# facebookresearch/vggsfm

Hardware: AMD Instinct MI355X
Metric: BA LM-iterations/sec (higher is better)
Workload: dtype f64

## Files before the change

vggsfm_amd/csrc/ba.hip:

```cpp
#include <type_traits>

#include "camera_model.hpp"
#include "../../include/vggsfm_amd.h"

namespace vgg {

int cholesky_solve_enqueue(double* A, double* b, int n, double* inv_blocks, int32_t* device_fail, const int32_t* skip_flag,
                           hipStream_t st, const CholOverlap* overlap, int split_a, int split_b, const int32_t* first_blk,
                           bool flags_cleared);
int32_t* cholesky_dataflow_flags(double* ws, int n, size_t* count);
size_t cholesky_workspace_bytes(int n);
void dataflow_signal(int32_t* flag, hipStream_t st);

constexpr int kGroup = 16;
#ifndef VGG_OFFDIAG_OCC
#define VGG_OFFDIAG_OCC 3
#endif
#ifndef VGG_DIAG_OCC
#define VGG_DIAG_OCC 4
#endif
#ifndef VGG_TILE_INTERLEAVE
#define VGG_TILE_INTERLEAVE 1
#endif
#ifndef VGG_DIAG_FULL_DEPTH
// ... 59 lines not shown
  double *scale_c, *scale_p, *colsq_c, *dsq_c, *dy;
  uint8_t* active;
  double* lin;
  double *U, *g, *costc;
  double* sys;
  double *S, *rhs;
  double* S2;
  double* gmax_pts;
  double* stepsum;
  double *G, *hs, *Ms;
  double *pdamp;
  double* T;
  double* part_B;
  double* part_F;
  double* packed;
  size_t packed_count;
  double* pk_mine;
  double* pk_gathered;
  double* cam_part;
  double* cam_split;
  double* Y;
  size_t y_bytes;
  double* chol_inv;
  double* tile_part;
  int32_t* batch_flags;
  double *Zp, *rz_part, *part_Q;
  unsigned long long* split_off;
  double* rz;
  int tile_rhs;
  int step_from_factors;
  double* Yx;
  size_t yx_bytes;
  int tile_dma;
  size_t lin_count, sys_count, total_bytes;
};

static inline size_t align_up(size_t x, size_t a) { return (x + a - 1) / a * a; }


static Dims make_dims(const vgg_ba_problem* pb) {
  Dims d;
  d.C = pb->num_cams; d.P = pb->num_pts; d.O = pb->num_obs; d.NI = pb->num_intr; d.model = pb->camera_model;
  const int rf = pb->refine_focal ? 1 : 0, rk = (pb->refine_extra && pb->camera_model == kSimpleRadial) ? 1 : 0;
  d.kd = rf + rk;
  d.only_k = (!rf && rk) ? 1 : 0;
  d.shared = (pb->num_intr == 1) ? 1 : 0;
  d.BDp = 6 + d.kd;
  d.n_red = 6 * d.C + d.kd * d.NI;
  d.kdsh = d.shared ? d.kd : 0;
  d.loss = pb->loss; d.loss_scale = pb->loss_scale;
  return d;
}

struct Tuning { int lpp, longt, cam_wgs, point_wgs, tile_rhs, step_factors, tile_dma; };
static Tuning g_tuning = [] {
  auto env = [](const char* name, int dflt) { const char* e = getenv(name); return e ? atoi(e) : dflt; };
  return Tuning{env("VGG_LPP", 0), env("VGG_PP_LONGT", -1), env("VGG_CAM_WGS", 0), env("VGG_POINT_WGS", 0), env("VGG_TILE_RHS", 2), env("VGG_STEP_FACTORS", 0), env("VGG_TILE_DMA", 0)};
}();

static Ws carve(const Dims& d, int max_iters, int num_chunks, int num_segments, void* base) {
  Ws w;
  size_t off = 0;
  auto take = [&](size_t bytes) { size_t o = off; off = align_up(off + bytes, 256); return (char*)base + o; };
  w.ctl = (Ctl*)take(sizeof(Ctl));
  w.log = (vgg_ba_iteration*)take(sizeof(vgg_ba_iteration) * (size_t)(max_iters + 2));
  w.cand_q = (double*)take(8ull * 4 * d.C); w.cand_t = (double*)take(8ull * 3 * d.C);
// ... 9 lines not shown
  w.sys = (double*)take(8ull * w.sys_count);
  w.S = w.sys; w.rhs = w.S + (size_t)d.n_red * d.n_red;
  w.S2 = (double*)take(8ull * (size_t)d.n_red * d.n_red);
  w.packed_count = (size_t)d.n_red * (d.n_red + 1) / 2 + d.n_red;
  w.packed = (double*)take(8ull * (w.packed_count + 2 * kPackPad));
  w.pk_mine = (double*)take(8ull * (w.packed_count + 2));
  w.pk_gathered = (double*)take(8ull * (w.packed_count + 3 * kPackPad));
  w.gmax_pts = (double*)take(64);
  w.stepsum = (double*)take(64);
  w.G = (double*)take(8ull * 6 * d.P); w.hs = (double*)take(8ull * 3 * d.P);
  w.pdamp = (double*)take(8ull * 3 * d.P);
  w.Ms = (double*)take(8ull * 3 * (d.kdsh ? d.kdsh : 1) * d.P);
  w.T = (double*)take(8ull * d.C * d.BDp * (1 + d.kdsh));
  w.part_B = (double*)take(8ull * kMaxWG);
  w.part_F = (double*)take(8ull * kMaxWG * 4);
  w.cam_part = (double*)take(8ull * (d.C + 1) * 3);
  w.cam_split = (double*)take(8ull * (size_t)d.C * kCamSplitMax * kCamNV);
  w.y_bytes = 8ull * ((size_t)(num_segments > 0 ? num_segments : 0) + 1) * kGroup * y_slot_doubles(d);
  w.Y = (double*)take(w.y_bytes);
  w.yx_bytes = (g_tuning.tile_dma && (d.shared || d.kd == 0)) ? 8ull * ((size_t)(num_segments > 0 ? num_segments : 0) + 1) * kGroup * 18 : 0;
  w.Yx = w.yx_bytes ? (double*)take(w.yx_bytes) : nullptr;
  w.tile_dma = 0;
  w.chol_inv = (double*)take(cholesky_workspace_bytes(d.n_red));
  {
    const size_t bdt = d.shared ? 6 : d.BDp;
    w.tile_part = (double*)take(8ull * (size_t)(num_chunks > 0 ? num_chunks : 1) * bdt * bdt * 256);
  }
  w.batch_flags = (int32_t*)take(64);
  w.Zp = (double*)take(8ull * 9 * (d.P > 0 ? d.P : 1));
  w.rz_part = (double*)take(8ull * (size_t)(num_chunks > 0 ? num_chunks : 1) * kGroup * 6 * 3);
  w.part_Q = (double*)take(8ull * kMaxWG * 8);
  w.rz = (double*)take(8ull * (size_t)((d.C + kGroup - 1) / kGroup) * kGroup * 6 * 3);
  w.split_off = (unsigned long long*)take(8ull * 2 * ((size_t)d.n_red + 2));
  w.tile_rhs = 0;
  w.total_bytes = off;
  return w;
}

struct DevProblem {
  Dims d;
  const double *cam_q, *cam_t, *intr, *pts;
  const int32_t *row_ptr, *obs_cam, *col_ptr, *cobs_pt, *obs_slot;
  const float2 *obs_uv, *cobs_uv;
  const uint8_t *cam_const, *intr_const, *pt_const;
};

static DevProblem dev_problem(const vgg_ba_problem* pb, const Dims& d) {
  DevProblem p;
  p.d = d; p.cam_q = pb->cam_q; p.cam_t = pb->cam_t; p.intr = pb->intr; p.pts = pb->pts;
  p.row_ptr = pb->row_ptr; p.obs_cam = pb->obs_cam; p.col_ptr = pb->col_ptr; p.cobs_pt = pb->cobs_pt;
  p.obs_slot = pb->obs_slot;
  p.obs_uv = (const float2*)pb->obs_uv; p.cobs_uv = (const float2*)pb->cobs_uv;
  p.cam_const = pb->cam_const; p.intr_const = pb->intr_const; p.pt_const = pb->pt_const;
  return p;
}

template <int N>
struct ObsPf {
  static_assert(N == 2 || N == 4, "prefetch depth");
  int c0 = 0, c1 = 0, c2 = 0, c3 = 0, s0 = 0, s1 = 0, s2 = 0, s3 = 0;
  float2 u0 = make_float2(0.f, 0.f), u1 = make_float2(0.f, 0.f), u2 = make_float2(0.f, 0.f), u3 = make_float2(0.f, 0.f);
  template <bool SLOT>
  __device__ __forceinline__ void load(const int32_t* cam, const float2* uv, const int32_t* slot, int o0, int o1, int stride, int sl) {
    int o = o0 + sl;
    if (o < o1) { c0 = cam[o]; u0 = uv[o]; if (SLOT) s0 = slot[o]; }
    o += stride;
// ... 107 lines not shown
      if (k >= 3 && (f & (2u << (k - 3)))) act = false;
    } else {
      const int a = (j - 6 * d.C) / d.kd;
      act = !(pb.intr_const && pb.intr_const[a]);
      if (!d.shared && world == 1 && !(pb.col_ptr[a + 1] > pb.col_ptr[a])) act = false;
    }
    w.active[j] = act ? 1 : 0;
    w.scale_c[j] = 1.0;
  }
}

__device__ __forceinline__ void zero_system_lower(const Ws& w, int n, int wg, int nwg) {
  const bool even = (n & 1) == 0;
  for (int row = wg; row <= n; row += nwg) {
    const int len = (row < n) ? min(n, 64 * (row / 64 + 1)) : n;
    double* dst = w.sys + (size_t)row * n;
    if (even) {
      double2* d2 = reinterpret_cast<double2*>(dst);
      for (int c = threadIdx.x; c < (len + 1) / 2; c += 256) d2[c] = make_double2(0.0, 0.0);
    } else {
      for (int c = threadIdx.x; c < len; c += 256) dst[c] = 0.0;
    }
  }
}

template <int KD, int MODE>
__global__ __launch_bounds__(256, (MODE == 1) ? VGG_CP_OCC_RHS : VGG_CP_OCC) void cam_pass_kernel(DevProblem pb, Ws w) {
  constexpr int BD = 6 + KD;
  constexpr int NU = BD * (BD + 1) / 2;
  constexpr int NV = (MODE == 0) ? (NU + BD + 1) : (BD * (1 + KD));
  __shared__ double red[4 * NV];
  __shared__ double tot[NV];
  if (w.ctl->done) return;
  if (MODE == 0 && !w.ctl->need_lin) return;
  if (MODE == 1) {
    zero_system_lower(w, pb.d.n_red, (int)(blockIdx.y * gridDim.x + blockIdx.x), (int)(gridDim.x * gridDim.y));
  }
  const Dims& d = pb.d;
  const int c = blockIdx.x, split = gridDim.y;
  double q[9], t[3], in4[4];
  quat_to_R(pb.cam_q + 4 * c, q);
#pragma unroll
  for (int k = 0; k < 3; ++k) t[k] = pb.cam_t[3 * c + k];
  const int a = d.shared ? 0 : c;
#pragma unroll
  for (int k = 0; k < 4; ++k) in4[k] = pb.intr[4 * a + k];
  const unsigned camflag = pb.cam_const ? pb.cam_const[c] : 0u;
  const bool intr_c = pb.intr_const ? pb.intr_const[a] != 0 : false;
  const int kdsh = d.kdsh;
  double acc[NV];
#pragma unroll
  for (int i = 0; i < NV; ++i) acc[i] = 0.0;
  const int j_begin = pb.col_ptr[c], j_count = pb.col_ptr[c + 1] - j_begin;
  const int per = (j_count + split - 1) / split;
  const int j0 = j_begin + (int)blockIdx.y * per, j1 = min(j0 + per, j_begin + j_count);
  constexpr int KM = (KD > 0) ? KD : 1;
  struct Gathered { double X[3], h[3], M[3 * KM]; float2 uv; int c; };
  auto gather = [&](Gathered& g, int p, float2 uv) __attribute__((always_inline)) {
    g.uv = uv;
    g.X[0] = pb.pts[3 * p]; g.X[1] = pb.pts[3 * p + 1]; g.X[2] = pb.pts[3 * p + 2];
    g.c = pb.pt_const ? (int)pb.pt_const[p] : 0;
    if (MODE == 1) {
      g.h[0] = w.hs[3 * p]; g.h[1] = w.hs[3 * p + 1]; g.h[2] = w.hs[3 * p + 2];
#pragma unroll
      for (int m = 0; m < KD; ++m)
        if (m < kdsh) {
          const double* M = w.Ms + ((size_t)p * kdsh + m) * 3;
// ... 32 lines not shown
        for (int k = i; k < BD; ++k) acc[u++] += F[i] * F[k] + F[BD + i] * F[BD + k];
#pragma unroll
      for (int i = 0; i < BD; ++i) acc[NU + i] += F[i] * r[0] + F[BD + i] * r[1];
      acc[NU + BD] += rho0;
    } else {
      double R0[1 + KD], R1[1 + KD];
      R0[0] = r[0] - (E[0] * h0 + E[1] * h1v + E[2] * h2);
      R1[0] = r[1] - (E[3] * h0 + E[4] * h1v + E[5] * h2);
#pragma unroll
      for (int m = 0; m < KD; ++m) {
        if (m < kdsh) {
          const double* M = Mc + 3 * m;
          R0[1 + m] = -(E[0] * M[0] + E[1] * M[1] + E[2] * M[2]);
          R1[1 + m] = -(E[3] * M[0] + E[4] * M[1] + E[5] * M[2]);
        } else { R0[1 + m] = 0; R1[1 + m] = 0; }
      }
#pragma unroll
      for (int i = 0; i < BD; ++i)
#pragma unroll
        for (int m = 0; m < 1 + KD; ++m) acc[i * (1 + KD) + m] += F[i] * R0[m] + F[BD + i] * R1[m];
    }
  }
  block_sum<NV>(acc, red, tot);
  static_assert(NV <= kCamNV, "cam_split row");
  if (threadIdx.x < NV) w.cam_split[((size_t)c * kCamSplitMax + blockIdx.y) * kCamNV + threadIdx.x] = tot[threadIdx.x];
}

template <int KD, int MODE>
__global__ __launch_bounds__(64) void cam_reduce_kernel(DevProblem pb, Ws w, int split, int point_parts) {
  constexpr int BD = 6 + KD;
  constexpr int NU = BD * (BD + 1) / 2;
  constexpr int NV = (MODE == 0) ? (NU + BD + 1) : (BD * (1 + KD));
  if (w.ctl->done) return;
  if (MODE == 0 && !w.ctl->need_lin) return;
  if (MODE == 1 && blockIdx.x == 0) {
    double m = 0;
    for (int i = threadIdx.x; i < point_parts; i += 64) m = fmax(m, w.part_B[i]);
    m = wave_max(m);
    if (threadIdx.x == 0) w.gmax_pts[0] = m;
  }
  const Dims& d = pb.d;
  const int c = blockIdx.x, kdsh = d.kdsh;
  if (threadIdx.x >= NV) return;
  double tot = 0.0;
#pragma unroll 8
  for (int sp = 0; sp < split; ++sp) tot += w.cam_split[((size_t)c * kCamSplitMax + sp) * kCamNV + threadIdx.x];
  if (MODE == 0) {
    double* U = w.U + (size_t)c * BD * BD;
    if (threadIdx.x < NU) {
      int i = 0, rem = threadIdx.x;
      while (rem >= BD - i) { rem -= BD - i; ++i; }
      const int k = i + rem;
      U[i * BD + k] = tot;
      U[k * BD + i] = tot;
    } else if (threadIdx.x < NU + BD) {
      w.g[(size_t)c * BD + threadIdx.x - NU] = tot;
    } else {
      w.costc[c] = tot;
    }
  } else {
    const int i = threadIdx.x / (1 + KD), m = threadIdx.x - i * (1 + KD);
    if (m < 1 + kdsh) w.T[((size_t)c * BD + i) * (1 + kdsh) + m] = tot;
  }
}

template <int KD>
__device__ __forceinline__ void prep_body(const DevProblem& pb, const Ws& w, const vgg_ba_options& opt, double* red) {
// ... 1437 lines not shown
    }
    const bool intr_var = KD > 0 && !(pb.intr_const && pb.intr_const[a]);
    const int np = (d.model == kSimpleRadial) ? 4 : 3;
    for (int k = 0; k < 4; ++k) { w.cand_intr[4 * a + k] = in4[k]; if (intr_var && k < np) xn += pb.intr[4 * a + k] * pb.intr[4 * a + k]; }
  }
  double mc = 0.0;
  if (c < d.C && w.step_from_factors) {
    constexpr int BD = 6 + KD;
    double dv[BD];
    for (int k = 0; k < 6; ++k) dv[k] = w.active[6 * c + k] ? w.scale_c[6 * c + k] * w.rhs[6 * c + k] : 0.0;
    const int ai = d.shared ? 0 : c;
    for (int k = 0; k < KD; ++k) { const int j = 6 * d.C + KD * ai + k; dv[6 + k] = w.active[j] ? w.scale_c[j] * w.rhs[j] : 0.0; }
    const double* U = w.U + (size_t)c * BD * BD;
    const double* g = w.g + (size_t)c * BD;
    double lin = 0.0, quad = 0.0;
    for (int i = 0; i < BD; ++i) {
      double ui = 0.0;
      for (int k = 0; k < BD; ++k) ui += U[i * BD + k] * dv[k];
      quad += dv[i] * ui;
      lin += dv[i] * g[i];
    }
    mc = lin - 0.5 * quad;
  }
  w.cam_part[3 * c] = step;
  w.cam_part[3 * c + 1] = xn;
  w.cam_part[3 * c + 2] = mc;
}

template <int KD, bool LDSCAM, int LPP, bool LONGT = false, int FYM = 0>
__global__ __launch_bounds__(256, FYM == 1 ? VGG_PS_OCC_FY : VGG_PS_OCC) void point_step_kernel(DevProblem pb, Ws w) {
  constexpr bool FY = FYM == 1;
  constexpr bool HY = FYM == 2;
  constexpr int BD = 6 + KD;
  __shared__ double red[4][4];
  extern __shared__ double cam_cache[];
  if (w.ctl->done) return;
  const Dims& d = pb.d;
  constexpr int PPW = 64 / LPP;
  const int wave = threadIdx.x >> 6, lane = threadIdx.x & 63;
  const int sub = lane / LPP, sl = lane % LPP;
  const int nw = gridDim.x * 4 * PPW;
  double s_cost = 0, s_mcc = 0, s_step = 0, s_xn = 0;
  const double* lq = cam_cache;
  const double* lt = lq + (FY ? 0 : 9 * d.C);
  const double* ldy = lt + (FY ? 0 : 3 * d.C);
  const double* lcq = ldy + 6 * d.C;
  const double* lct = lcq + 9 * d.C;
  const double* lfl = lct + 3 * d.C;
  if (LDSCAM) {
    double* cc = cam_cache;
    for (int i = threadIdx.x; i < d.C; i += 256) {
      if (!FY) {
        quat_to_R(pb.cam_q + 4 * i, cc + 9 * i);
        cc[30 * d.C + i] = pb.cam_const ? (double)pb.cam_const[i] : 0.0;
      }
      quat_to_R(w.cand_q + 4 * i, cc + (lcq - cam_cache) + 9 * i);
    }
    for (int i = threadIdx.x; i < 3 * d.C; i += 256) { if (!FY) cc[9 * d.C + i] = pb.cam_t[i]; cc[(lct - cam_cache) + i] = w.cand_t[i]; }
    for (int i = threadIdx.x; i < 6 * d.C; i += 256) cc[(ldy - cam_cache) + i] = w.dy[i];
    __syncthreads();
  }
  (void)lfl;
  int p = (blockIdx.x * 4 + wave) * PPW + sub;
  constexpr int NPF = LONGT ? 4 : 2;
  int n_o0 = 0, n_o1 = 0;
  ObsPf<NPF> n_pf;
  double n_X0 = 0, n_X1 = 0, n_X2 = 0;
  int n_ptc = 0;
  int m_o0 = 0, m_o1 = 0;
  double m_X0 = 0, m_X1 = 0, m_X2 = 0;
  int m_ptc = 0;
  if (p < d.P) {
    n_o0 = pb.row_ptr[p]; n_o1 = pb.row_ptr[p + 1];
    n_X0 = pb.pts[3 * p]; n_X1 = pb.pts[3 * p + 1]; n_X2 = pb.pts[3 * p + 2];
    n_ptc = pb.pt_const ? (int)pb.pt_const[p] : 0;
    n_pf.template load<(FYM != 0)>(pb.obs_cam, pb.obs_uv, pb.obs_slot, n_o0, n_o1, LPP, sl);
    if (p + nw < d.P) {
      const int pm = p + nw;
      m_o0 = pb.row_ptr[pm]; m_o1 = pb.row_ptr[pm + 1];
      m_X0 = pb.pts[3 * pm]; m_X1 = pb.pts[3 * pm + 1]; m_X2 = pb.pts[3 * pm + 2];
      m_ptc = pb.pt_const ? (int)pb.pt_const[pm] : 0;
    }
  }
  for (; p < d.P; p += nw) {
    const int o0 = n_o0, o1 = n_o1;
    const double X[3] = {n_X0, n_X1, n_X2};
    const bool pt_c = n_ptc != 0;
    const ObsPf<NPF> f_pf = n_pf;
    {
      n_o0 = m_o0; n_o1 = m_o1; n_X0 = m_X0; n_X1 = m_X1; n_X2 = m_X2; n_ptc = m_ptc;
      if (p + nw < d.P) n_pf.template load<(FYM != 0)>(pb.obs_cam, pb.obs_uv, pb.obs_slot, n_o0, n_o1, LPP, sl);
// ... 38 lines not shown
      double fy0 = 0, fy1 = 0;
#pragma unroll
      for (int k = 0; k < 6; ++k) { const double v = LDSCAM ? ldy[6 * c + k] : w.dy[6 * c + k]; fy0 += F[k] * v; fy1 += F[BD + k] * v; }
      if (!HY) {
#pragma unroll
        for (int k = 0; k < KD; ++k) { const double v = w.dy[6 * d.C + KD * a + k]; fy0 += F[6 + k] * v; fy1 += F[BD + 6 + k] * v; }
      }
      t3[0] += E[0] * fy0 + E[3] * fy1; t3[1] += E[1] * fy0 + E[4] * fy1; t3[2] += E[2] * fy0 + E[5] * fy1;
      if (!HY) s_mcc += fy0 * (r[0] - 0.5 * fy0) + fy1 * (r[1] - 0.5 * fy1);
    };
    for (int o = o0 + sl; o < o1; o += LPP) {
      const int pass = (o - o0) / LPP;
      if (FY || (HY && (pass & 1))) from_factor(pass, o);
      else evaluated(pass, o);
    }
#pragma unroll
    for (int i = 0; i < 3; ++i) t3[i] = group_sum<LPP>(t3[i]);
    double u0 = 0, u1 = 0, u2 = 0;
    if (!FY) { u0 = G00 * t3[0]; u1 = G01 * t3[0] + G11 * t3[1]; u2 = G02 * t3[0] + G12 * t3[1] + G22 * t3[2]; }
    if (FYM != 0) { u0 += group_sum<LPP>(uf[0]); u1 += group_sum<LPP>(uf[1]); u2 += group_sum<LPP>(uf[2]); }
    double ys[3];
    ys[0] = hs0 - (G00 * u0 + G01 * u1 + G02 * u2);
    ys[1] = hs1 - (G11 * u1 + G12 * u2);
    ys[2] = hs2 - (G22 * u2);
    if constexpr (FYM != 0 && KD > 0) {
      const double* Msp = w.Ms + (size_t)p * 3 * KD;
#pragma unroll
      for (int m = 0; m < KD; ++m) {
        const int j = 6 * d.C + m;
        const double ds = w.active[j] ? w.rhs[j] : 0.0;
        ys[0] -= Msp[3 * m] * ds; ys[1] -= Msp[3 * m + 1] * ds; ys[2] -= Msp[3 * m + 2] * ds;
      }
    }
    const double Xn[3] = {X[0] - ys[0], X[1] - ys[1], X[2] - ys[2]};
    if (sl == 0) {
      w.cand_pts[3 * (size_t)p] = Xn[0]; w.cand_pts[3 * (size_t)p + 1] = Xn[1]; w.cand_pts[3 * (size_t)p + 2] = Xn[2];
      s_step += ys[0] * ys[0] + ys[1] * ys[1] + ys[2] * ys[2];
      if (!pt_c) s_xn += X[0] * X[0] + X[1] * X[1] + X[2] * X[2];
      if (G22 != 0.0) {
        const double z2 = ys[2] / G22, z1 = (ys[1] - G12 * z2) / G11, z0 = (ys[0] - G01 * z1 - G02 * z2) / G00;
        s_mcc += 0.5 * (z0 * z0 + z1 * z1 + z2 * z2) + 0.5 * (pd0 * ys[0] * ys[0] + pd1 * ys[1] * ys[1] + pd2 * ys[2] * ys[2]);
      }
    }
    for (int o = o0 + sl; o < o1; o += LPP) {
      const int pass = (o - o0) / LPP;
      const int c = f_pf.cam(pass, pb.obs_cam, o);
      const int a = d.shared ? 0 : c;
      const float2 uv = f_pf.uv(pass, pb.obs_uv, o);
      double rc[2];
      if (LDSCAM) obs_residual_R(d.model, lcq + 9 * c, lct + 3 * c, w.cand_intr + 4 * a, Xn, (double)uv.x, (double)uv.y, rc);
      else obs_residual_R(d.model, CamR(w.cand_q + 4 * c).R, w.cand_t + 3 * c, w.cand_intr + 4 * a, Xn, (double)uv.x, (double)uv.y, rc);
      s_cost += loss_rho0(d, rc[0] * rc[0] + rc[1] * rc[1]);
    }
  }
  s_cost = wave_sum(s_cost); s_mcc = wave_sum(s_mcc); s_step = wave_sum(s_step); s_xn = wave_sum(s_xn);
  if (lane == 0) { red[wave][0] = s_cost; red[wave][1] = s_mcc; red[wave][2] = s_step; red[wave][3] = s_xn; }
  __syncthreads();
  if (threadIdx.x < 4) w.part_F[4 * blockIdx.x + threadIdx.x] = red[0][threadIdx.x] + red[1][threadIdx.x] + red[2][threadIdx.x] + red[3][threadIdx.x];
}

__global__ __launch_bounds__(256) void reduce_step_kernel(Ws w, int nparts) {
  __shared__ double red[4][256];
  if (w.ctl->done) return;
  double s[4] = {0, 0, 0, 0};
  for (int i = threadIdx.x; i < nparts; i += 256)
    for (int k = 0; k < 4; ++k) s[k] += w.part_F[4 * i + k];
  for (int k = 0; k < 4; ++k) red[k][threadIdx.x] = s[k];
  __syncthreads();
  for (int st = 128; st > 0; st >>= 1) {
    if (threadIdx.x < st) for (int k = 0; k < 4; ++k) red[k][threadIdx.x] += red[k][threadIdx.x + st];
    __syncthreads();
  }
  if (threadIdx.x < 4) w.stepsum[threadIdx.x] = red[threadIdx.x][0];
}

__global__ __launch_bounds__(64) void control_kernel(Ws w, vgg_ba_options opt, int C) {
  Ctl* c = w.ctl;
  if (c->done) { if (threadIdx.x == 0) c->accept = 0; return; }
  double step_c = 0, xn_c = 0, mcc_c = 0;
#pragma unroll 4
  for (int i = threadIdx.x; i <= C; i += 64) { step_c += w.cam_part[3 * i]; xn_c += w.cam_part[3 * i + 1]; mcc_c += w.cam_part[3 * i + 2]; }
  step_c = wave_sum(step_c); xn_c = wave_sum(xn_c); mcc_c = wave_sum(mcc_c);
  if (threadIdx.x != 0) return;
  const int it = c->iteration;
  vgg_ba_iteration li;
  li.iteration = it; li.successful = 0; li.cost = c->x_cost; li.cost_change = 0; li.gradient_max_norm = c->gmax;
  li.step_norm = 0; li.relative_decrease = 0; li.radius = c->radius;
  c->accept = 0;
  const double cand_cost = 0.5 * w.stepsum[0];
  const double mcc = w.stepsum[1] + mcc_c;
  const double step_norm = sqrt(w.stepsum[2] + step_c);
  const double x_norm = sqrt(w.stepsum[3] + xn_c);
  c->cand_cost = cand_cost; c->mcc = mcc; c->step_norm = step_norm;
  const bool step_valid = !c->linear_fail && (mcc > 0.0);
  c->linear_fail = 0;
  if (!step_valid) {
    if (++c->invalid_streak >= opt.max_num_consecutive_invalid_steps) { c->done = 1; c->termination = 5; }
    c->radius /= c->decrease_factor; c->decrease_factor *= 2.0;
    c->num_unsucc += 1;
    li.radius = c->radius;
    w.log[it] = li;
    return;
  }
  c->invalid_streak = 0;
  li.step_norm = step_norm;
  li.cost_change = c->x_cost - cand_cost;
  const double ptol = opt.parameter_tolerance * (x_norm + opt.parameter_tolerance);
  if (!(step_norm > ptol)) { c->done = 1; c->termination = 3; w.log[it] = li; return; }
  if (fabs(c->x_cost - cand_cost) <= opt.function_tolerance * c->x_cost) { c->done = 1; c->termination = 2; w.log[it] = li; return; }
  const double rel = (c->x_cost - cand_cost) / mcc;
  c->rel = rel;
  li.relative_decrease = rel;
  if (rel > opt.min_relative_decrease) {
    c->accept = 1;
    c->x_cost = cand_cost;
    const double tmp = 2.0 * rel - 1.0;
    c->radius = c->radius / fmax(1.0 / 3.0, 1.0 - tmp * tmp * tmp);
    c->radius = fmin(opt.max_trust_region_radius, c->radius);
    c->decrease_factor = 2.0;
    c->need_lin = 1;
    c->num_succ += 1;
    li.successful = 1; li.cost = cand_cost;
  } else {
    c->radius /= c->decrease_factor; c->decrease_factor *= 2.0;
    c->num_unsucc += 1;
  }
  li.radius = c->radius;
  w.log[it] = li;
}

__global__ void commit_kernel(Ws w, double* cam_q, double* cam_t, double* intr, double* pts, int C, int NI, int P) {
  if (!w.ctl->accept) return;
  const size_t i = (size_t)blockIdx.x * blockDim.x + threadIdx.x;
  if (i < (size_t)3 * P) pts[i] = w.cand_pts[i];
  if (i < (size_t)4 * C) cam_q[i] = w.cand_q[i];
  if (i < (size_t)3 * C) cam_t[i] = w.cand_t[i];
  if (i < (size_t)4 * NI) intr[i] = w.cand_intr[i];
}

enum { kProfLinearize = 0, kProfPointPass, kProfCamRhs, kProfSchurTile, kProfCholesky, kProfPointStep,
       kProfSchurTileDiag, kProfCount };
struct Profiler {
  bool on = false;
  int cap = 0;
  hipEvent_t* start[kProfCount] = {};
  hipEvent_t* stop[kProfCount] = {};
  int n[kProfCount] = {};
};
static Profiler g_prof;
struct ProfScope {
  int id; hipStream_t st; bool live;
  ProfScope(int id_, hipStream_t st_) : id(id_), st(st_), live(g_prof.on && g_prof.n[id_] < g_prof.cap) {
    if (live) (void)hipEventRecord(g_prof.start[id][g_prof.n[id]], st);
  }
  ~ProfScope() {
    if (live) { (void)hipEventRecord(g_prof.stop[id][g_prof.n[id]], st); g_prof.n[id]++; }
  }
};

struct Launch {
  Dims d; DevProblem dp; Ws w; vgg_ba_options opt; hipStream_t st; int wgB;
  int lpp;
  const int32_t* chunk_desc; const int32_t* entries; int num_chunks, num_segments;
  int merged_tile_launch;
  const int32_t* tile_desc; int num_tiles;
  const int32_t* batches; int num_batches;
// ... 104 lines not shown
  if (i == n) {
    if (mode == 0) {
      for (size_t j = total + threadIdx.x; j < W * chunk; j += 256) packed[j] = 0.0;
      if (part == 1 && threadIdx.x == 0) w.pk_mine[chunk_a + chunk_b] = w.gmax_pts[0];
    } else if (part == 1 && threadIdx.x < 64) {
      double m = 0.0;
      for (size_t r = threadIdx.x; r < W; r += 64) m = fmax(m, gathered[r * gstride + chunk]);
      m = wave_max(m);
      if (threadIdx.x == 0) w.gmax_pts[0] = m;
    }
  }
}
static size_t split_count_a(const Dims& d) {
  size_t c = 0;
  const int P6 = 6 * d.C, GW = 6 * kGroup;
  for (int r = 0; r < d.n_red; ++r) {
    if (r < P6) c += (size_t)GW * (r / GW);
    else if (!(d.shared || d.kd == 0)) {
      const int a = (r - P6) / d.kd, g = a / kGroup;
      const int pb0 = GW * g, pb1 = (GW * (g + 1) < P6) ? GW * (g + 1) : P6;
      c += (size_t)pb0 + (size_t)(P6 - pb1) + (size_t)kGroup * d.kd * g;
    }
  }
  return c;
}

static inline int cam_split_for(int C, int O) {
  const int target = g_tuning.cam_wgs > 0 ? g_tuning.cam_wgs : min(1024, max(256, O / 2048));
  const int s = target / (C > 0 ? C : 1);
  return s < 1 ? 1 : (s > kCamSplitMax ? kCamSplitMax : s);
}

template <int KD>
static void phase_linearize(const Launch& L) {
  ProfScope ps(kProfLinearize, L.st);
  const int split = cam_split_for(L.d.C, L.d.O);
  cam_pass_kernel<KD, 0><<<dim3(L.d.C, split), 256, 0, L.st>>>(L.dp, L.w);
  cam_reduce_kernel<KD, 0><<<L.d.C, 64, 0, L.st>>>(L.dp, L.w, split, 0);
}

template <int BD>
static void launch_schur_batch(const Launch& L, int batch, hipStream_t st, double* dst, int which = 0) {
  const int32_t* B = L.batches + 6 * batch;
  const int c0 = B[0], cm = B[1], c1 = B[2], t0 = B[3], t1 = B[4];
  if (L.merged_tile_launch && c1 > c0) {
    ProfScope ps(kProfSchurTile, st);
    schur_tile_merged_kernel<BD><<<c1 - c0, 256, 0, st>>>(L.w, L.chunk_desc, L.entries, c0, L.num_segments);
  } else if (cm > c0 && which != 2) {
    if (BD == 6 && L.w.tile_dma) {
      {
        ProfScope ps(kProfCamRhs, st);
        expand_segments_kernel<<<div_up((L.num_segments + 1) * kGroup, 256), 256, 0, st>>>(L.w, L.num_segments);
      }
      ProfScope ps(kProfSchurTile, st);
      if (L.w.tile_dma == 2) schur_tile_dma_kernel<2><<<cm - c0, 256, 0, st>>>(L.w, L.chunk_desc, L.entries, c0, L.num_segments);
      else schur_tile_dma_kernel<1><<<cm - c0, 256, 0, st>>>(L.w, L.chunk_desc, L.entries, c0, L.num_segments);
    } else {
      ProfScope ps(kProfSchurTile, st);
      schur_tile_kernel<BD, false><<<cm - c0, 256, 0, st>>>(L.w, L.chunk_desc, L.entries, c0, L.num_segments);
    }
  }
  if (!L.merged_tile_launch && c1 > cm && which != 1) {
    ProfScope ps(kProfSchurTileDiag, st);
    schur_tile_kernel<BD, true><<<c1 - cm, 256, 0, st>>>(L.w, L.chunk_desc, L.entries, cm, L.num_segments);
  }
  if (t1 > t0)
    tile_reduce_kernel<BD><<<dim3(div_up(kGroup * BD * kGroup * BD, 256) + (L.w.tile_rhs ? (BD == 6 ? div_up(kGroup * BD * 3, 256) : div_up(2 * kGroup * BD, 256)) : 0),
                                  t1 - t0), 256, 0, st>>>(L.w, L.d.n_red, L.d.C, L.d.kd, L.tile_desc, t0, dst, which == 0 ? -1 : which - 1);
}

template <int KD>
// ... 104 lines not shown
  begin_iteration_kernel<<<1, 256, 0, L.st>>>(L.w, L.opt, d.n_red, chol_flags, chol_flags ? (int)chol_flag_count : 0);
  int rc;
  if (OverlapCtx* oc = overlap_ctx(L)) {
    (void)hipMemsetAsync(L.w.batch_flags, 0, 64, L.st);
    (void)hipEventRecord(oc->ready, L.st);
    (void)hipStreamWaitEvent(oc->st_rest, oc->ready, 0);
    (void)hipStreamWaitEvent(oc->st_chol, oc->ready, 0);
    launch_schur_batches<KD>(L, 1, L.num_batches, oc->st_rest, L.w.S2, oc->batch_done, L.w.batch_flags);
    CholOverlap ov;
    ov.dev_flags = L.w.batch_flags + 1;
    ov.S2 = L.w.S2;
    ov.first_col = 6 * kGroup * L.batches[6 * 1 + 5];
    ov.num_waits = L.num_batches - 1;
    for (int b = 1; b < L.num_batches; ++b) {
      ov.wait_col[b - 1] = 6 * kGroup * L.batches[6 * b + 5];
      ov.wait_ev[b - 1] = oc->batch_done[b];
    }
    {
      ProfScope ps(kProfCholesky, oc->st_chol);
      rc = cholesky_solve_enqueue(L.w.S, L.w.rhs, d.n_red, L.w.chol_inv, &L.w.ctl->linear_fail, &L.w.ctl->done, oc->st_chol, &ov,
                                  L.chol_split_a, L.chol_split_b, L.chol_first_blk, chol_flags != nullptr);
    }
    (void)hipEventRecord(oc->chol_done, oc->st_chol);
    (void)hipStreamWaitEvent(L.st, oc->chol_done, 0);
  } else {
    ProfScope ps(kProfCholesky, L.st);
    rc = cholesky_solve_enqueue(L.w.S, L.w.rhs, d.n_red, L.w.chol_inv, &L.w.ctl->linear_fail, &L.w.ctl->done, L.st, nullptr,
                                L.chol_split_a, L.chol_split_b, L.chol_first_blk, chol_flags != nullptr);
  }
  if (rc != VGG_OK) return rc;
  cam_update_kernel<KD><<<div_up(d.C + 1, 64), 64, 0, L.st>>>(L.dp, L.w);
  {
    ProfScope ps(kProfPointStep, L.st);
    const size_t cam_lds = sizeof(double) * 31 * (size_t)d.C;
    auto launch = [&](auto lpp) {
      constexpr int LPP = decltype(lpp)::value;
      const bool longt = long_tracks(LPP, L.d.P, L.d.O);
      auto go = [&](auto fy) {
        constexpr int FY = decltype(fy)::value;
        const size_t lds = FY == 1 ? sizeof(double) * 18 * (size_t)d.C : cam_lds;
        if (longt && LPP <= 32) {
          if (lds <= 64 * 1024) point_step_kernel<KD, true, LPP, (LPP <= 32), FY><<<L.wgB, 256, lds, L.st>>>(L.dp, L.w);
          else point_step_kernel<KD, false, LPP, (LPP <= 32), FY><<<L.wgB, 256, 0, L.st>>>(L.dp, L.w);
        } else if (lds <= 64 * 1024) point_step_kernel<KD, true, LPP, false, FY><<<L.wgB, 256, lds, L.st>>>(L.dp, L.w);
        else point_step_kernel<KD, false, LPP, false, FY><<<L.wgB, 256, 0, L.st>>>(L.dp, L.w);
      };
      if (L.w.step_from_factors == 1) go(std::integral_constant<int, 1>{});
      else if (L.w.step_from_factors == 2) go(std::integral_constant<int, 2>{});
      else go(std::integral_constant<int, 0>{});
    };
    if (L.lpp == 8) launch(std::integral_constant<int, 8>{});
    else if (L.lpp == 16) launch(std::integral_constant<int, 16>{});
    else if (L.lpp == 32) launch(std::integral_constant<int, 32>{});
    else launch(std::integral_constant<int, 64>{});
  }
  reduce_step_kernel<<<1, 256, 0, L.st>>>(L.w, L.wgB);
  return VGG_OK;
}

static void phase_update(const Launch& L) {
  const Dims& d = L.d;
  control_kernel<<<1, 64, 0, L.st>>>(L.w, L.opt, d.C);
  size_t nmax = (size_t)3 * d.P;
  if ((size_t)4 * d.C > nmax) nmax = (size_t)4 * d.C;
  if ((size_t)4 * d.NI > nmax) nmax = (size_t)4 * d.NI;
  commit_kernel<<<div_up((long)nmax, 256), 256, 0, L.st>>>(L.w, L.cam_q, L.cam_t, L.intr, L.pts, d.C, d.NI, d.P);
}

static int device_cus() {
  static int cus[64] = {0};
  int dev = 0;
  if (hipGetDevice(&dev) != hipSuccess || dev < 0 || dev >= 64) return 256;
  if (cus[dev] == 0) {
    int n = 0;
    if (hipDeviceGetAttribute(&n, hipDeviceAttributeMultiprocessorCount, dev) != hipSuccess || n <= 0) n = 256;
    cus[dev] = n;
  }
  return cus[dev];
}

static int make_launch(const vgg_ba_problem* pb, const vgg_ba_options* opt, void* workspace, hipStream_t st, Launch* L) {
  if (!pb || !opt || !workspace) return VGG_ERR_INVALID_ARGUMENT;
  if (pb->num_cams <= 0 || pb->num_pts < 0 || pb->num_obs < 0) return VGG_ERR_INVALID_ARGUMENT;
  if (pb->num_intr != 1 && pb->num_intr != pb->num_cams) return VGG_ERR_UNSUPPORTED;
  if (pb->camera_model != kPinhole && pb->camera_model != kSimpleRadial) return VGG_ERR_UNSUPPORTED;
  L->d = make_dims(pb);
  L->dp = dev_problem(pb, L->d);
  L->w = carve(L->d, opt->max_num_iterations, pb->num_chunks, pb->num_segments, workspace);
  L->opt = *opt;
  L->st = st;
  L->lpp = lanes_per_point(L->d.P, L->d.O);
  L->wgB = min(max(div_up(L->d.P, 4 * (64 / L->lpp)), 1), g_tuning.point_wgs > 0 ? min(g_tuning.point_wgs, kMaxWG) : min(2 * device_cus(), kMaxWG));
  L->chunk_desc = pb->chunk_desc; L->entries = pb->entries; L->num_chunks = pb->num_chunks;
  L->merged_tile_launch = pb->merged_tile_launch;
  L->num_segments = pb->num_segments;
  L->batches = pb->tile_batches; L->num_batches = pb->num_tile_batches;
  L->chol_split_a = pb->chol_split_a; L->chol_split_b = pb->chol_split_b;
  L->chol_first_blk = pb->chol_first_blk;
  if (pb->chol_split_a < 0 || pb->chol_split_b < 0 || pb->chol_split_a % 64 != 0 ||
      pb->chol_split_a + pb->chol_split_b > 6 * pb->num_cams)
    return VGG_ERR_INVALID_ARGUMENT;
  if (pb->num_chunks > 0) {
    if (!pb->tile_batches || pb->num_tile_batches < 1) return VGG_ERR_INVALID_ARGUMENT;
    int prev_c = 0, prev_t = 0, prev_g = 0;
    for (int b = 0; b < pb->num_tile_batches; ++b) {
      const int32_t* B = pb->tile_batches + 6 * b;
      if (B[0] != prev_c || B[1] < B[0] || B[2] < B[1] || B[3] != prev_t || B[4] < B[3] || B[5] < prev_g) return VGG_ERR_INVALID_ARGUMENT;
      prev_c = B[2]; prev_t = B[4]; prev_g = B[5];
    }
    if (prev_c != pb->num_chunks || prev_t != pb->num_tiles) return VGG_ERR_INVALID_ARGUMENT;
  }
  L->tile_desc = pb->tile_desc; L->num_tiles = pb->num_tiles;
  L->w.tile_rhs = (g_tuning.tile_rhs && (L->d.shared || L->d.kd == 0 || g_tuning.tile_rhs >= 2) && pb->num_chunks > 0 &&
                   pb->num_tile_batches == 1) ? 1 : 0;
  L->w.step_from_factors = (L->d.shared || L->d.kd == 0) ? g_tuning.step_factors : 0;
  L->w.tile_dma = (L->w.Yx && !pb->merged_tile_launch && pb->num_tile_batches == 1) ? g_tuning.tile_dma : 0;
  L->cam_q = pb->cam_q; L->cam_t = pb->cam_t; L->intr = pb->intr; L->pts = pb->pts;
  return VGG_OK;
}

template <typename Fn0, typename Fn1, typename Fn2>
static int dispatch_kd(int kd, Fn0 f0, Fn1 f1, Fn2 f2) {
  switch (kd) { case 0: return f0(); case 1: return f1(); default: return f2(); }
}

static int run_phase(const Launch& L, int phase) {
  switch (phase) {
    case 0:
      return dispatch_kd(L.d.kd, [&] { phase_linearize<0>(L); return VGG_OK; }, [&] { phase_linearize<1>(L); return VGG_OK; },
                         [&] { phase_linearize<2>(L); return VGG_OK; });
    case 1:
      return dispatch_kd(L.d.kd, [&] { phase_schur<0>(L); return VGG_OK; }, [&] { phase_schur<1>(L); return VGG_OK; },
                         [&] { phase_schur<2>(L); return VGG_OK; });
    case 2:
      return dispatch_kd(L.d.kd, [&] { return phase_step<0>(L); }, [&] { return phase_step<1>(L); }, [&] { return phase_step<2>(L); });
    case 3: phase_update(L); return VGG_OK;
    case 4: pack_lower_kernel<<<L.d.n_red + 1, 256, 0, L.st>>>(L.w, L.d.n_red, 0); return VGG_OK;
    case 5: pack_lower_kernel<<<L.d.n_red + 1, 256, 0, L.st>>>(L.w, L.d.n_red, 1); return VGG_OK;
    case 6: pack_lower_kernel<<<L.d.n_red + 1, 256, 0, L.st>>>(L.w, L.d.n_red, 2); return VGG_OK;
    case 7: case 9: case 12:
      if (L.num_batches != 1 || L.merged_tile_launch || L.d.C <= kGroup) return VGG_ERR_UNSUPPORTED;
      if (phase == 12) {
        split_offsets_kernel<<<1, 256, 0, L.st>>>(L.w, L.d.n_red, L.d.C, L.d.kd, L.d.shared);
        return VGG_OK;
      }
      return dispatch_kd(L.d.kd, [&] { phase_schur<0>(L, phase == 7 ? 1 : 2); return VGG_OK; },
                         [&] { phase_schur<1>(L, phase == 7 ? 1 : 2); return VGG_OK; },
                         [&] { phase_schur<2>(L, phase == 7 ? 1 : 2); return VGG_OK; });
    case 8: case 10:
      pack_split_kernel<<<L.d.n_red + 1, 256, 0, L.st>>>(L.w, L.d.n_red, L.d.C, L.d.kd, L.d.shared, phase == 8 ? 0 : 1, 0);
      return VGG_OK;
    case 11:
      pack_split_kernel<<<L.d.n_red + 1, 256, 0, L.st>>>(L.w, L.d.n_red, L.d.C, L.d.kd, L.d.shared, 0, 2);
      pack_split_kernel<<<L.d.n_red + 1, 256, 0, L.st>>>(L.w, L.d.n_red, L.d.C, L.d.kd, L.d.shared, 1, 2);
      return VGG_OK;
    default: return VGG_ERR_INVALID_ARGUMENT;
  }
}

static int finish(const Launch& L, int max_iters, vgg_ba_summary* summary, vgg_ba_iteration* log, int log_cap) {
  Ctl h;
  if (hipMemcpyAsync(&h, L.w.ctl, sizeof(Ctl), hipMemcpyDeviceToHost, L.st) != hipSuccess) return VGG_ERR_HIP;
  int ncopy = 0;
// ... 75 lines not shown
  *total_ms = tot; *launches = g_prof.n[kernel_id];
  if (reset) g_prof.n[kernel_id] = 0;
  return VGG_OK;
}

const char* vgg_build_arch(void) { return "gfx950"; }
int vgg_abi_version(void) { return VGG_ABI_VERSION; }
size_t vgg_abi_sizeof(int which) {
  switch (which) {
    case 0: return sizeof(vgg_ba_problem);
    case 1: return sizeof(vgg_ba_options);
    case 2: return sizeof(vgg_ba_iteration);
    case 3: return sizeof(vgg_ba_summary);
    default: return 0;
  }
}

size_t vgg_ba_workspace_bytes(const vgg_ba_problem* problem, const vgg_ba_options* options) {
  if (!problem || !options) return 0;
  const Dims d = make_dims(problem);
  return carve(d, options->max_num_iterations, problem->num_chunks, problem->num_segments, nullptr).total_bytes + 256;
}

int vgg_ba_begin(const vgg_ba_problem* problem, const vgg_ba_options* options, void* workspace, size_t workspace_bytes,
                 int rank, int world_size, void* stream) {
  Launch L;
  int rc = make_launch(problem, options, workspace, (hipStream_t)stream, &L);
  if (rc != VGG_OK) return rc;
  if (workspace_bytes < L.w.total_bytes) return VGG_ERR_WORKSPACE;
  if (world_size < 1 || world_size > kPackPad || rank < 0 || rank >= world_size) return VGG_ERR_INVALID_ARGUMENT;
  VGG_HIP_CHECK(hipMemsetAsync(L.w.Y, 0, L.w.y_bytes, L.st));
  VGG_HIP_CHECK(hipMemsetAsync(L.w.sys, 0, sizeof(double) * L.w.sys_count, L.st));
  init_kernel<<<div_up(L.d.n_red > 0 ? L.d.n_red : 1, 256), 256, 0, L.st>>>(L.dp, L.w, L.opt, rank, world_size);
  VGG_LAUNCH_CHECK();
  return VGG_OK;
}

int vgg_ba_phase(const vgg_ba_problem* problem, const vgg_ba_options* options, void* workspace, int phase, void* stream) {
  Launch L;
  int rc = make_launch(problem, options, workspace, (hipStream_t)stream, &L);
  if (rc != VGG_OK) return rc;
  rc = run_phase(L, phase);
  if (rc != VGG_OK) return rc;
  VGG_LAUNCH_CHECK();
  return VGG_OK;
}

int vgg_ba_reduce_buffer(const vgg_ba_problem* problem, const vgg_ba_options* options, void* workspace, int which,
                         double** device_ptr, size_t* count) {
  if (!problem || !options || !workspace || !device_ptr || !count) return VGG_ERR_INVALID_ARGUMENT;
  const Dims d = make_dims(problem);
  Ws w = carve(d, options->max_num_iterations, problem->num_chunks, problem->num_segments, workspace);
  switch (which) {
    case 0: *device_ptr = w.lin; *count = w.lin_count; break;
    case 1: *device_ptr = w.sys; *count = w.sys_count; break;
    case 2: *device_ptr = w.gmax_pts; *count = 1; break;
    case 3: *device_ptr = w.stepsum; *count = 4; break;
    case 4: *device_ptr = w.packed; *count = w.packed_count; break;
    case 5: *device_ptr = w.pk_mine; *count = w.packed_count + 2; break;
    case 6: *device_ptr = w.pk_gathered; *count = w.packed_count + 3 * kPackPad; break;
    case 7: *device_ptr = w.packed; *count = split_count_a(d); break;
    default: return VGG_ERR_INVALID_ARGUMENT;
  }
  return VGG_OK;
}

// ... 53 lines not shown
```

Before: 690.6.

## Linearize at candidate during step phase and commit linearization on accept

Candidate cost evaluation moves out of the point step kernel. The step phase now runs the camera linearization passes at the candidate parameters into a separate buffer, and that buffer also supplies the candidate cost. On accept, the commit kernel copies the candidate linearization into the live buffers, so the separate linearize phase becomes a no-op and the initial linearization happens in begin. This removes a whole linearize pass per iteration and the per-observation cost recompute, at the price of linearizing even for rejected steps, an extra copy of the linearization buffer, and more workspace.

```diff
diff --git a/vggsfm_amd/csrc/ba.hip b/vggsfm_amd/csrc/ba.hip
--- a/vggsfm_amd/csrc/ba.hip
+++ b/vggsfm_amd/csrc/ba.hip
@@ -115,6 +115,8 @@
   double* Yx;
   size_t yx_bytes;
   int tile_dma;
+  double* lin_cand;
+  double *U_cand, *g_cand, *cost_cand;
   size_t lin_count, sys_count, total_bytes;
 };
 
@@ -190,6 +192,8 @@
   w.part_Q = (double*)take(8ull * kMaxWG * 8);
   w.rz = (double*)take(8ull * (size_t)((d.C + kGroup - 1) / kGroup) * kGroup * 6 * 3);
   w.split_off = (unsigned long long*)take(8ull * 2 * ((size_t)d.n_red + 2));
+  w.lin_cand = (double*)take(8ull * w.lin_count);
+  w.U_cand = w.lin_cand; w.g_cand = w.U_cand + (size_t)d.C * d.BDp * d.BDp; w.cost_cand = w.g_cand + (size_t)d.C * d.BDp;
   w.tile_rhs = 0;
   w.total_bytes = off;
   return w;
@@ -363,7 +367,6 @@
   __shared__ double red[4 * NV];
   __shared__ double tot[NV];
   if (w.ctl->done) return;
-  if (MODE == 0 && !w.ctl->need_lin) return;
   if (MODE == 1) {
     zero_system_lower(w, pb.d.n_red, (int)(blockIdx.y * gridDim.x + blockIdx.x), (int)(gridDim.x * gridDim.y));
   }
@@ -462,7 +465,6 @@
   constexpr int NU = BD * (BD + 1) / 2;
   constexpr int NV = (MODE == 0) ? (NU + BD + 1) : (BD * (1 + KD));
   if (w.ctl->done) return;
-  if (MODE == 0 && !w.ctl->need_lin) return;
   if (MODE == 1 && blockIdx.x == 0) {
     double m = 0;
     for (int i = threadIdx.x; i < point_parts; i += 64) m = fmax(m, w.part_B[i]);
@@ -1966,7 +1968,7 @@
   constexpr bool FY = FYM == 1;
   constexpr bool HY = FYM == 2;
   constexpr int BD = 6 + KD;
-  __shared__ double red[4][4];
+  __shared__ double red[4][3];
   extern __shared__ double cam_cache[];
   if (w.ctl->done) return;
   const Dims& d = pb.d;
@@ -1974,23 +1976,20 @@
   const int wave = threadIdx.x >> 6, lane = threadIdx.x & 63;
   const int sub = lane / LPP, sl = lane % LPP;
   const int nw = gridDim.x * 4 * PPW;
-  double s_cost = 0, s_mcc = 0, s_step = 0, s_xn = 0;
+  double s_mcc = 0, s_step = 0, s_xn = 0;
   const double* lq = cam_cache;
   const double* lt = lq + (FY ? 0 : 9 * d.C);
   const double* ldy = lt + (FY ? 0 : 3 * d.C);
-  const double* lcq = ldy + 6 * d.C;
-  const double* lct = lcq + 9 * d.C;
-  const double* lfl = lct + 3 * d.C;
+  const double* lfl = ldy + 6 * d.C;
   if (LDSCAM) {
     double* cc = cam_cache;
-    for (int i = threadIdx.x; i < d.C; i += 256) {
-      if (!FY) {
+    if (!FY) {
+      for (int i = threadIdx.x; i < d.C; i += 256) {
         quat_to_R(pb.cam_q + 4 * i, cc + 9 * i);
-        cc[30 * d.C + i] = pb.cam_const ? (double)pb.cam_const[i] : 0.0;
-      }
-      quat_to_R(w.cand_q + 4 * i, cc + (lcq - cam_cache) + 9 * i);
-    }
-    for (int i = threadIdx.x; i < 3 * d.C; i += 256) { if (!FY) cc[9 * d.C + i] = pb.cam_t[i]; cc[(lct - cam_cache) + i] = w.cand_t[i]; }
+        cc[18 * d.C + i] = pb.cam_const ? (double)pb.cam_const[i] : 0.0;
+      }
+      for (int i = threadIdx.x; i < 3 * d.C; i += 256) cc[9 * d.C + i] = pb.cam_t[i];
+    }
     for (int i = threadIdx.x; i < 6 * d.C; i += 256) cc[(ldy - cam_cache) + i] = w.dy[i];
     __syncthreads();
   }
@@ -2095,9 +2094,8 @@
         ys[0] -= Msp[3 * m] * ds; ys[1] -= Msp[3 * m + 1] * ds; ys[2] -= Msp[3 * m + 2] * ds;
       }
     }
-    const double Xn[3] = {X[0] - ys[0], X[1] - ys[1], X[2] - ys[2]};
     if (sl == 0) {
-      w.cand_pts[3 * (size_t)p] = Xn[0]; w.cand_pts[3 * (size_t)p + 1] = Xn[1]; w.cand_pts[3 * (size_t)p + 2] = Xn[2];
+      w.cand_pts[3 * (size_t)p] = X[0] - ys[0]; w.cand_pts[3 * (size_t)p + 1] = X[1] - ys[1]; w.cand_pts[3 * (size_t)p + 2] = X[2] - ys[2];
       s_step += ys[0] * ys[0] + ys[1] * ys[1] + ys[2] * ys[2];
       if (!pt_c) s_xn += X[0] * X[0] + X[1] * X[1] + X[2] * X[2];
       if (G22 != 0.0) {
@@ -2105,29 +2103,20 @@
         s_mcc += 0.5 * (z0 * z0 + z1 * z1 + z2 * z2) + 0.5 * (pd0 * ys[0] * ys[0] + pd1 * ys[1] * ys[1] + pd2 * ys[2] * ys[2]);
       }
     }
-    for (int o = o0 + sl; o < o1; o += LPP) {
-      const int pass = (o - o0) / LPP;
-      const int c = f_pf.cam(pass, pb.obs_cam, o);
-      const int a = d.shared ? 0 : c;
-      const float2 uv = f_pf.uv(pass, pb.obs_uv, o);
-      double rc[2];
-      if (LDSCAM) obs_residual_R(d.model, lcq + 9 * c, lct + 3 * c, w.cand_intr + 4 * a, Xn, (double)uv.x, (double)uv.y, rc);
-      else obs_residual_R(d.model, CamR(w.cand_q + 4 * c).R, w.cand_t + 3 * c, w.cand_intr + 4 * a, Xn, (double)uv.x, (double)uv.y, rc);
-      s_cost += loss_rho0(d, rc[0] * rc[0] + rc[1] * rc[1]);
-    }
-  }
-  s_cost = wave_sum(s_cost); s_mcc = wave_sum(s_mcc); s_step = wave_sum(s_step); s_xn = wave_sum(s_xn);
-  if (lane == 0) { red[wave][0] = s_cost; red[wave][1] = s_mcc; red[wave][2] = s_step; red[wave][3] = s_xn; }
+  }
+  s_mcc = wave_sum(s_mcc); s_step = wave_sum(s_step); s_xn = wave_sum(s_xn);
+  if (lane == 0) { red[wave][0] = s_mcc; red[wave][1] = s_step; red[wave][2] = s_xn; }
   __syncthreads();
-  if (threadIdx.x < 4) w.part_F[4 * blockIdx.x + threadIdx.x] = red[0][threadIdx.x] + red[1][threadIdx.x] + red[2][threadIdx.x] + red[3][threadIdx.x];
-}
-
-__global__ __launch_bounds__(256) void reduce_step_kernel(Ws w, int nparts) {
+  if (threadIdx.x < 3) w.part_F[4 * blockIdx.x + 1 + threadIdx.x] = red[0][threadIdx.x] + red[1][threadIdx.x] + red[2][threadIdx.x] + red[3][threadIdx.x];
+}
+
+__global__ __launch_bounds__(256) void reduce_step_kernel(Ws w, int nparts, int C) {
   __shared__ double red[4][256];
   if (w.ctl->done) return;
   double s[4] = {0, 0, 0, 0};
+  for (int i = threadIdx.x; i < C; i += 256) s[0] += w.cost_cand[i];
   for (int i = threadIdx.x; i < nparts; i += 256)
-    for (int k = 0; k < 4; ++k) s[k] += w.part_F[4 * i + k];
+    for (int k = 1; k < 4; ++k) s[k] += w.part_F[4 * i + k];
   for (int k = 0; k < 4; ++k) red[k][threadIdx.x] = s[k];
   __syncthreads();
   for (int st = 128; st > 0; st >>= 1) {
@@ -2193,8 +2182,13 @@
 }
 
 __global__ void commit_kernel(Ws w, double* cam_q, double* cam_t, double* intr, double* pts, int C, int NI, int P) {
-  if (!w.ctl->accept) return;
+  const Ctl* ctl = w.ctl;
   const size_t i = (size_t)blockIdx.x * blockDim.x + threadIdx.x;
+  if (!ctl->accept) {
+    if (ctl->world > 1 && ctl->rank != 0 && i < w.lin_count) w.lin[i] = 0.0;
+    return;
+  }
+  if (i < w.lin_count) w.lin[i] = w.lin_cand[i];
   if (i < (size_t)3 * P) pts[i] = w.cand_pts[i];
   if (i < (size_t)4 * C) cam_q[i] = w.cand_q[i];
   if (i < (size_t)3 * C) cam_t[i] = w.cand_t[i];
@@ -2365,11 +2359,10 @@
 }
 
 template <int KD>
-static void phase_linearize(const Launch& L) {
-  ProfScope ps(kProfLinearize, L.st);
+static void launch_linearize(const Launch& L, const DevProblem& dp, const Ws& w) {
   const int split = cam_split_for(L.d.C, L.d.O);
-  cam_pass_kernel<KD, 0><<<dim3(L.d.C, split), 256, 0, L.st>>>(L.dp, L.w);
-  cam_reduce_kernel<KD, 0><<<L.d.C, 64, 0, L.st>>>(L.dp, L.w, split, 0);
+  cam_pass_kernel<KD, 0><<<dim3(L.d.C, split), 256, 0, L.st>>>(dp, w);
+  cam_reduce_kernel<KD, 0><<<L.d.C, 64, 0, L.st>>>(dp, w, split, 0);
 }
 
 template <int BD>
@@ -2540,13 +2533,13 @@
   cam_update_kernel<KD><<<div_up(d.C + 1, 64), 64, 0, L.st>>>(L.dp, L.w);
   {
     ProfScope ps(kProfPointStep, L.st);
-    const size_t cam_lds = sizeof(double) * 31 * (size_t)d.C;
+    const size_t cam_lds = sizeof(double) * 19 * (size_t)d.C;
     auto launch = [&](auto lpp) {
       constexpr int LPP = decltype(lpp)::value;
       const bool longt = long_tracks(LPP, L.d.P, L.d.O);
       auto go = [&](auto fy) {
         constexpr int FY = decltype(fy)::value;
-        const size_t lds = FY == 1 ? sizeof(double) * 18 * (size_t)d.C : cam_lds;
+        const size_t lds = FY == 1 ? sizeof(double) * 6 * (size_t)d.C : cam_lds;
         if (longt && LPP <= 32) {
           if (lds <= 64 * 1024) point_step_kernel<KD, true, LPP, (LPP <= 32), FY><<<L.wgB, 256, lds, L.st>>>(L.dp, L.w);
           else point_step_kernel<KD, false, LPP, (LPP <= 32), FY><<<L.wgB, 256, 0, L.st>>>(L.dp, L.w);
@@ -2562,7 +2555,15 @@
     else if (L.lpp == 32) launch(std::integral_constant<int, 32>{});
     else launch(std::integral_constant<int, 64>{});
   }
-  reduce_step_kernel<<<1, 256, 0, L.st>>>(L.w, L.wgB);
+  {
+    ProfScope ps(kProfLinearize, L.st);
+    DevProblem dc = L.dp;
+    dc.cam_q = L.w.cand_q; dc.cam_t = L.w.cand_t; dc.intr = L.w.cand_intr; dc.pts = L.w.cand_pts;
+    Ws wc = L.w;
+    wc.U = L.w.U_cand; wc.g = L.w.g_cand; wc.costc = L.w.cost_cand;
+    launch_linearize<KD>(L, dc, wc);
+  }
+  reduce_step_kernel<<<1, 256, 0, L.st>>>(L.w, L.wgB, d.C);
   return VGG_OK;
 }
 
@@ -2572,6 +2573,7 @@
   size_t nmax = (size_t)3 * d.P;
   if ((size_t)4 * d.C > nmax) nmax = (size_t)4 * d.C;
   if ((size_t)4 * d.NI > nmax) nmax = (size_t)4 * d.NI;
+  if (L.w.lin_count > nmax) nmax = L.w.lin_count;
   commit_kernel<<<div_up((long)nmax, 256), 256, 0, L.st>>>(L.w, L.cam_q, L.cam_t, L.intr, L.pts, d.C, d.NI, d.P);
 }
 
@@ -2634,9 +2636,7 @@
 
 static int run_phase(const Launch& L, int phase) {
   switch (phase) {
-    case 0:
-      return dispatch_kd(L.d.kd, [&] { phase_linearize<0>(L); return VGG_OK; }, [&] { phase_linearize<1>(L); return VGG_OK; },
-                         [&] { phase_linearize<2>(L); return VGG_OK; });
+    case 0: return VGG_OK;
     case 1:
       return dispatch_kd(L.d.kd, [&] { phase_schur<0>(L); return VGG_OK; }, [&] { phase_schur<1>(L); return VGG_OK; },
                          [&] { phase_schur<2>(L); return VGG_OK; });
@@ -2778,6 +2778,8 @@
   VGG_HIP_CHECK(hipMemsetAsync(L.w.Y, 0, L.w.y_bytes, L.st));
   VGG_HIP_CHECK(hipMemsetAsync(L.w.sys, 0, sizeof(double) * L.w.sys_count, L.st));
   init_kernel<<<div_up(L.d.n_red > 0 ? L.d.n_red : 1, 256), 256, 0, L.st>>>(L.dp, L.w, L.opt, rank, world_size);
+  (void)dispatch_kd(L.d.kd, [&] { launch_linearize<0>(L, L.dp, L.w); return VGG_OK; },
+                    [&] { launch_linearize<1>(L, L.dp, L.w); return VGG_OK; }, [&] { launch_linearize<2>(L, L.dp, L.w); return VGG_OK; });
   VGG_LAUNCH_CHECK();
   return VGG_OK;
 }
```

New measurement: 701.9 (median of 6 runs). +1.6%, better.
